# agent-charon/MinGraph-UNet

Hardware: AMD Instinct MI355X
Metric: segmented Mpix/sec, full MinGraph-UNet forward (U-Net + patch-graph GAT), 512x512 batch (higher is better)
Workload: dtype f32

## Files before the change

mingraph-unet_amd/csrc/convt_x3.hip:

```cpp
#include <hip/hip_runtime.h>
#include <stdint.h>

#include <algorithm>
#include <type_traits>

#include "common.h"
#include "pack_small.h"

namespace mgu {

typedef float f32x16 __attribute__((ext_vector_type(16)));
typedef float f32x4 __attribute__((ext_vector_type(4)));
typedef unsigned u32x4 __attribute__((ext_vector_type(4)));
typedef __bf16 bf16x8 __attribute__((ext_vector_type(8)));

namespace {

__device__ __forceinline__ void split3_pack(const float a, const float b, unsigned& p0, unsigned& p1, unsigned& p2) {
  const unsigned ua = __float_as_uint(a), ub = __float_as_uint(b);
  p0 = __builtin_amdgcn_perm(ub, ua, 0x07060302u);
  const float ra = a - __uint_as_float(ua & 0xffff0000u), rb = b - __uint_as_float(ub & 0xffff0000u);
  const unsigned va = __float_as_uint(ra), vb = __float_as_uint(rb);
  p1 = __builtin_amdgcn_perm(vb, va, 0x07060302u);
  const float sa = ra - __uint_as_float(va & 0xffff0000u), sb = rb - __uint_as_float(vb & 0xffff0000u);
  p2 = __builtin_amdgcn_perm(__float_as_uint(sb), __float_as_uint(sa), 0x07060302u);
}

__device__ __forceinline__ f32x16 mfma_bf16(const u32x4 a, const u32x4 b, const f32x16 c) {
  return __builtin_amdgcn_mfma_f32_32x32x16_bf16(__builtin_bit_cast(bf16x8, a), __builtin_bit_cast(bf16x8, b), c, 0, 0, 0);
}

__global__ void pack_convt_x3_kernel(const float* __restrict__ w, uint16_t* __restrict__ Wx, int Cin, int Cout) {
  pack_convt_x3_body(w, Wx, Cin, Cout, 0, blockIdx.x, gridDim.x);
}

__device__ __forceinline__ void lds_barrier() { asm volatile("s_waitcnt lgkmcnt(0)\n\ts_barrier" ::: "memory"); }

template <int MODE, int NI>
__global__ __launch_bounds__(256, 2) void convt2x2_x3_kernel(const float* __restrict__ in, const int ldin, const uint16_t* __restrict__ Wx,
                                                             const float* __restrict__ shift, float* __restrict__ out, const int M,
                                                             const int H, const int W, const int Cin, const int Cout, const int ldout,
                                                             const int coff, const int Hout, const int Wout, const int ntn,
                                                             const int nblocks) {
  constexpr int AP = 40, ABUF = 3 * 128 * AP;
  __shared__ __attribute__((aligned(16))) uint16_t As[2 * ABUF];
  __shared__ int rowoff[128];
  const int chunk = gridDim.x >> 3;
  const int lb = (blockIdx.x & 7) * chunk + (blockIdx.x >> 3);
  if (lb >= nblocks) return;
  const int nt = lb % ntn, mt = lb / ntn;
  const int tid = threadIdx.x, lane = tid & 63, wave = tid >> 6;
  const int wm = wave >> 1, wn = wave & 1, lr = lane & 31, lh = lane >> 5;
  const int bm0 = mt * 128;
  const int HW = H * W;
  long long pix0;
  {
    const int img = bm0 / HW, rem = bm0 - img * HW, y = rem / W;
    pix0 = ((long long)img * Hout + 2 * y) * Wout + 2 * (rem - y * W);
  }
  if (tid < 128) {
    const int m = bm0 + tid;
    int off = 0;
    if (m < M) {
      const int img = m / HW, rem = m - img * HW, y = rem / W, x = rem - y * W;
      off = (int)((((long long)img * Hout + 2 * y) * Wout + 2 * x - pix0) * ldout);
    }
    rowoff[tid] = off;
  }

  const int arow = tid >> 3, ach = (tid & 7) * 4;
  const float* aptr[4];
#pragma unroll
  for (int j = 0; j < 4; ++j) {
    const int m = min(bm0 + j * 32 + arow, M - 1);
    if (MODE == 0) {
      aptr[j] = in + (size_t)m * ldin + ach;
    } else {
      const int img = m / HW, rem = m - img * HW, y = rem / W, x = rem - y * W;
      aptr[j] = in + (((size_t)img * Hout + 2 * y) * Wout + 2 * x) * ldin + ach;
    }
  }
  const int nk = (MODE == 0 ? Cin : 4 * Cin) >> 5;
  const int spq = Cin >> 5;
  auto koff = [&](int s) -> int {
    if (MODE == 0) return s * 32;
    const int q = s / spq;
    return ((q >> 1) * Wout + (q & 1)) * ldin + (s - q * spq) * 32;
  };
  f32x4 areg[2][4];
  auto load_a = [&](int s, auto set_t) {
    constexpr int set = decltype(set_t)::value;
    const int ko = koff(s);
#pragma unroll
    for (int j = 0; j < 4; ++j) areg[set][j] = *reinterpret_cast<const f32x4*>(aptr[j] + ko);
  };
  auto store_a = [&](int buf, auto set_t) {
    constexpr int set = decltype(set_t)::value;
    uint16_t* const base = As + buf * ABUF + arow * AP + ach;
#pragma unroll
    for (int j = 0; j < 4; ++j) {
      unsigned p[3][2];
      split3_pack(areg[set][j][0], areg[set][j][1], p[0][0], p[1][0], p[2][0]);
      split3_pack(areg[set][j][2], areg[set][j][3], p[0][1], p[1][1], p[2][1]);
#pragma unroll
      for (int q = 0; q < 3; ++q) *reinterpret_cast<uint2*>(base + (q * 128 + j * 32) * AP) = uint2{p[q][0], p[q][1]};
    }
  };

  const int nt128 = NI == 2 ? nt : nt >> 1, sub0 = NI == 2 ? wn * 2 : (nt & 1) * 2 + wn;
  const u32x4* const bp = reinterpret_cast<const u32x4*>(Wx) + ((size_t)nt128 * (2 * nk) * 12 + sub0 * 3) * 64 + lane;
  u32x4 br[2][3 * NI];
  auto load_b = [&](int kk, auto buf_t) {
    constexpr int buf = decltype(buf_t)::value;
#pragma unroll
    for (int f = 0; f < 3 * NI; ++f) br[buf][f] = bp[((size_t)kk * 12 + f) * 64];
  };

  f32x16 acc[2][NI];
#pragma unroll
  for (int mi = 0; mi < 2; ++mi)
#pragma unroll
    for (int ni = 0; ni < NI; ++ni)
#pragma unroll
      for (int r = 0; r < 16; ++r) acc[mi][ni][r] = 0.f;

  const int aoff = (wm * 64 + lr) * AP + lh * 8;
  auto half_step = [&](int buf, int ss, auto bb_t) {
    constexpr int bb = decltype(bb_t)::value;
    u32x4 pa[2][3];
#pragma unroll
    for (int mi = 0; mi < 2; ++mi)
#pragma unroll
      for (int q = 0; q < 3; ++q)
        pa[mi][q] = *reinterpret_cast<const u32x4*>(As + buf * ABUF + (q * 128 + mi * 32) * AP + aoff + ss * 16);
#pragma unroll
    for (int mi = 0; mi < 2; ++mi)
#pragma unroll
      for (int ni = 0; ni < NI; ++ni) {
        f32x16 t = acc[mi][ni];
        t = mfma_bf16(pa[mi][2], br[bb][ni * 3 + 0], t);
        t = mfma_bf16(pa[mi][0], br[bb][ni * 3 + 2], t);
        t = mfma_bf16(pa[mi][1], br[bb][ni * 3 + 1], t);
        t = mfma_bf16(pa[mi][1], br[bb][ni * 3 + 0], t);
        t = mfma_bf16(pa[mi][0], br[bb][ni * 3 + 1], t);
        t = mfma_bf16(pa[mi][0], br[bb][ni * 3 + 0], t);
        acc[mi][ni] = t;
      }
  };
  using B0 = std::integral_constant<int, 0>;
  using B1 = std::integral_constant<int, 1>;
  const int nkk = 2 * nk;
  load_a(0, B0{});
  load_a(min(1, nk - 1), B1{});
  load_b(0, B0{});
  store_a(0, B0{});
  lds_barrier();
  auto second_half_and_stage = [&](int buf, auto bb_t, auto set_t) {
    half_step(buf, 1, bb_t);
    store_a(buf ^ 1, set_t);
#pragma unroll
    for (int k = 0; k < 12 * NI; ++k) {
      __builtin_amdgcn_sched_group_barrier(0x008, 1, 0);
      __builtin_amdgcn_sched_group_barrier(0x002, NI == 2 ? 4 : 8, 0);
    }
    __builtin_amdgcn_sched_group_barrier(0x200, 12, 0);
  };
  for (int s = 0; s < nk; s += 2) {
    load_a(min(s + 2, nk - 1), B0{});
    load_b(min(2 * s + 1, nkk - 1), B1{});
    __builtin_amdgcn_sched_barrier(0);
    half_step(0, 0, B0{});
    load_b(min(2 * s + 2, nkk - 1), B0{});
    __builtin_amdgcn_sched_barrier(0);
    second_half_and_stage(0, B1{}, B1{});
    __builtin_amdgcn_sched_barrier(0);
    lds_barrier();
    if (s + 1 >= nk) break;
    load_a(min(s + 3, nk - 1), B1{});
    load_b(min(2 * s + 3, nkk - 1), B1{});
    __builtin_amdgcn_sched_barrier(0);
    half_step(1, 0, B0{});
    load_b(min(2 * s + 4, nkk - 1), B0{});
    __builtin_amdgcn_sched_barrier(0);
    second_half_and_stage(1, B1{}, B0{});
    __builtin_amdgcn_sched_barrier(0);
    lds_barrier();
  }

  float* const tile_out = MODE == 0 ? out + (size_t)pix0 * ldout + coff : out + (size_t)bm0 * ldout + coff;
  const bool full_m = bm0 + 128 <= M;
  auto store_tile = [&](auto guarded_t) {
    constexpr bool GUARDED = decltype(guarded_t)::value;
#pragma unroll
    for (int ni = 0; ni < NI; ++ni) {
      const int n = nt * (64 * NI) + wn * (32 * NI) + ni * 32 + lr;
      int ncol = n;
      if (MODE == 0) {
        const int q = n / Cout;
        ncol = ((q >> 1) * Wout + (q & 1)) * ldout + (n - q * Cout);
      }
      const float sh = shift ? shift[n] : 0.f;
#pragma unroll
      for (int mi = 0; mi < 2; ++mi)
#pragma unroll
        for (int r = 0; r < 16; ++r) {
          const int rrow = wm * 64 + mi * 32 + (r & 3) + 8 * (r >> 2) + 4 * lh;
          const unsigned idx = (unsigned)((MODE == 0 ? rowoff[rrow] : rrow * ldout) + ncol);
          const float v = acc[mi][ni][r] + sh;
          if (!GUARDED) tile_out[idx] = v;
          else if (bm0 + rrow < M) tile_out[idx] = v;
        }
    }
  };
  if (full_m) store_tile(std::false_type{});
  else store_tile(std::true_type{});
}

}

size_t convt_x3_floats(int Cin, int Cout) { return (size_t)Cin * Cout * 6; }


namespace {

__global__ void pack_convt_x3_dgrad_kernel(const float* __restrict__ w, uint16_t* __restrict__ Wx, int Cin, int Cout) {
  pack_convt_x3_body(w, Wx, Cin, Cout, 1, blockIdx.x, gridDim.x);
}

}

size_t convt_x3_dgrad_floats(int Cin, int Cout) { return (size_t)((Cin + 127) / 128 * 128) * Cout * 6; }

hipError_t launch_pack_convt_x3_dgrad(const float* w, float* Wx, int Cin, int Cout, hipStream_t s) {
  if ((Cin & 63) || (Cout & 31)) return hipErrorInvalidValue;
  hipLaunchKernelGGL(pack_convt_x3_dgrad_kernel, dim3((unsigned)std::min<int64_t>(4096, ((int64_t)Cin * Cout * 4 + 255) / 256)), dim3(256), 0, s, w,
                     reinterpret_cast<uint16_t*>(Wx), Cin, Cout);
  return hipGetLastError();
}

hipError_t launch_convt_x3_dgrad(const IgemmDesc& d, hipStream_t s) {
  const bool wide = (d.N & 127) == 0;
  const int mtiles = (d.M + 127) / 128, ntn = d.N / (wide ? 128 : 64);
  const int nb = mtiles * ntn;
  const int chunk = (nb + 7) / 8;
  if (wide)
    hipLaunchKernelGGL((convt2x2_x3_kernel<1, 2>), dim3(chunk * 8), dim3(256), 0, s, d.in, d.ldin, reinterpret_cast<const uint16_t*>(d.wu),
                       (const float*)nullptr, d.out, d.M, d.H, d.W, d.Cp, d.N, d.ldout, d.coff, d.Hout, d.Wout, ntn, nb);
  else
    hipLaunchKernelGGL((convt2x2_x3_kernel<1, 1>), dim3(chunk * 8), dim3(256), 0, s, d.in, d.ldin, reinterpret_cast<const uint16_t*>(d.wu),
                       (const float*)nullptr, d.out, d.M, d.H, d.W, d.Cp, d.N, d.ldout, d.coff, d.Hout, d.Wout, ntn, nb);
  return hipGetLastError();
}

hipError_t launch_pack_convt_x3(const float* w, float* Wx, int Cin, int Cout, hipStream_t s) {
  if ((Cin & 15) || (Cout & 31)) return hipErrorInvalidValue;
  hipLaunchKernelGGL(pack_convt_x3_kernel, dim3((unsigned)std::min<int64_t>(4096, ((int64_t)Cin * Cout * 4 + 255) / 256)), dim3(256), 0, s, w, reinterpret_cast<uint16_t*>(Wx), Cin,
                     Cout);
  return hipGetLastError();
}

hipError_t launch_convt_x3(const IgemmDesc& d, hipStream_t s) {
  const int mtiles = (d.M + 127) / 128, ntn = d.N / 128;
  const int nb = mtiles * ntn;
  const int chunk = (nb + 7) / 8;
  hipLaunchKernelGGL((convt2x2_x3_kernel<0, 2>), dim3(chunk * 8), dim3(256), 0, s, d.in, d.ldin, reinterpret_cast<const uint16_t*>(d.wu), d.shift, d.out,
                     d.M, d.H, d.W, d.Cp, d.ct_cout, d.ldout, d.coff, d.Hout, d.Wout, ntn, nb);
  return hipGetLastError();
}

}
```

Baseline: 800.3.

## Make MODE-0 transposed-conv kernel persistent with prefetch of next tile during epilogue

The MODE-0 transposed-conv GEMM kernel becomes persistent. The grid is capped at about two workgroups per CU, and each workgroup walks tiles with a stride of gridDim. While the current tile's output is being stored, the next tile's A and B prologue loads and its A staging are issued. Row offsets are double-buffered in LDS, and B loads are shifted later within each step. The aim is to hide prologue latency and remove per-tile launch and tail overhead, at the cost of more register pressure and more complex control flow.

After: 801.4 (median of 6 runs). About the same (+0.1%).

```diff
diff --git a/mingraph-unet_amd/csrc/convt_x3.hip b/mingraph-unet_amd/csrc/convt_x3.hip
--- a/mingraph-unet_amd/csrc/convt_x3.hip
+++ b/mingraph-unet_amd/csrc/convt_x3.hip
@@ -2,6 +2,7 @@
 #include <stdint.h>
 
 #include <algorithm>
+#include <atomic>
 #include <type_traits>
 
 #include "common.h"
@@ -42,46 +43,54 @@
                                                              const int H, const int W, const int Cin, const int Cout, const int ldout,
                                                              const int coff, const int Hout, const int Wout, const int ntn,
                                                              const int nblocks) {
+  constexpr bool WALK = MODE == 0;
   constexpr int AP = 40, ABUF = 3 * 128 * AP;
   __shared__ __attribute__((aligned(16))) uint16_t As[2 * ABUF];
-  __shared__ int rowoff[128];
+  __shared__ int rowoff[WALK ? 2 : 1][128];
   const int chunk = gridDim.x >> 3;
-  const int lb = (blockIdx.x & 7) * chunk + (blockIdx.x >> 3);
+  int lb = (blockIdx.x & 7) * chunk + (blockIdx.x >> 3);
   if (lb >= nblocks) return;
-  const int nt = lb % ntn, mt = lb / ntn;
   const int tid = threadIdx.x, lane = tid & 63, wave = tid >> 6;
   const int wm = wave >> 1, wn = wave & 1, lr = lane & 31, lh = lane >> 5;
-  const int bm0 = mt * 128;
   const int HW = H * W;
-  long long pix0;
-  {
-    const int img = bm0 / HW, rem = bm0 - img * HW, y = rem / W;
-    pix0 = ((long long)img * Hout + 2 * y) * Wout + 2 * (rem - y * W);
-  }
-  if (tid < 128) {
-    const int m = bm0 + tid;
-    int off = 0;
-    if (m < M) {
-      const int img = m / HW, rem = m - img * HW, y = rem / W, x = rem - y * W;
-      off = (int)((((long long)img * Hout + 2 * y) * Wout + 2 * x - pix0) * ldout);
-    }
-    rowoff[tid] = off;
-  }
-
   const int arow = tid >> 3, ach = (tid & 7) * 4;
-  const float* aptr[4];
-#pragma unroll
-  for (int j = 0; j < 4; ++j) {
-    const int m = min(bm0 + j * 32 + arow, M - 1);
-    if (MODE == 0) {
-      aptr[j] = in + (size_t)m * ldin + ach;
-    } else {
-      const int img = m / HW, rem = m - img * HW, y = rem / W, x = rem - y * W;
-      aptr[j] = in + (((size_t)img * Hout + 2 * y) * Wout + 2 * x) * ldin + ach;
-    }
-  }
   const int nk = (MODE == 0 ? Cin : 4 * Cin) >> 5;
   const int spq = Cin >> 5;
+
+  int nt, bm0;
+  long long pix0;
+  const float* aptr[4];
+  const u32x4* bp;
+  auto start_tile = [&](const int t, const int rb) {
+    nt = __builtin_amdgcn_readfirstlane(t % ntn);
+    bm0 = __builtin_amdgcn_readfirstlane((t / ntn) * 128);
+    {
+      const int img = bm0 / HW, rem = bm0 - img * HW, y = rem / W;
+      pix0 = ((long long)img * Hout + 2 * y) * Wout + 2 * (rem - y * W);
+    }
+    if (tid < 128) {
+      const int m = bm0 + tid;
+      int off = 0;
+      if (m < M) {
+        const int img = m / HW, rem = m - img * HW, y = rem / W, x = rem - y * W;
+        off = (int)((((long long)img * Hout + 2 * y) * Wout + 2 * x - pix0) * ldout);
+      }
+      rowoff[rb][tid] = off;
+    }
+#pragma unroll
+    for (int j = 0; j < 4; ++j) {
+      const int m = min(bm0 + j * 32 + arow, M - 1);
+      if (MODE == 0) {
+        aptr[j] = in + (size_t)m * ldin + ach;
+      } else {
+        const int img = m / HW, rem = m - img * HW, y = rem / W, x = rem - y * W;
+        aptr[j] = in + (((size_t)img * Hout + 2 * y) * Wout + 2 * x) * ldin + ach;
+      }
+    }
+    const int nt128 = NI == 2 ? nt : nt >> 1, sub0 = NI == 2 ? wn * 2 : (nt & 1) * 2 + wn;
+    bp = reinterpret_cast<const u32x4*>(Wx) + ((size_t)nt128 * (2 * nk) * 12 + sub0 * 3) * 64 + lane;
+  };
+
   auto koff = [&](int s) -> int {
     if (MODE == 0) return s * 32;
     const int q = s / spq;
@@ -107,8 +116,6 @@
     }
   };
 
-  const int nt128 = NI == 2 ? nt : nt >> 1, sub0 = NI == 2 ? wn * 2 : (nt & 1) * 2 + wn;
-  const u32x4* const bp = reinterpret_cast<const u32x4*>(Wx) + ((size_t)nt128 * (2 * nk) * 12 + sub0 * 3) * 64 + lane;
   u32x4 br[2][3 * NI];
   auto load_b = [&](int kk, auto buf_t) {
     constexpr int buf = decltype(buf_t)::value;
@@ -117,13 +124,6 @@
   };
 
   f32x16 acc[2][NI];
-#pragma unroll
-  for (int mi = 0; mi < 2; ++mi)
-#pragma unroll
-    for (int ni = 0; ni < NI; ++ni)
-#pragma unroll
-      for (int r = 0; r < 16; ++r) acc[mi][ni][r] = 0.f;
-
   const int aoff = (wm * 64 + lr) * AP + lh * 8;
   auto half_step = [&](int buf, int ss, auto bb_t) {
     constexpr int bb = decltype(bb_t)::value;
@@ -150,11 +150,12 @@
   using B0 = std::integral_constant<int, 0>;
   using B1 = std::integral_constant<int, 1>;
   const int nkk = 2 * nk;
-  load_a(0, B0{});
-  load_a(min(1, nk - 1), B1{});
-  load_b(0, B0{});
-  store_a(0, B0{});
-  lds_barrier();
+  auto load_first = [&]() {
+    load_a(0, B0{});
+    load_a(min(1, nk - 1), B1{});
+    load_b(0, B0{});
+    if (WALK) load_b(1, B1{});
+  };
   auto second_half_and_stage = [&](int buf, auto bb_t, auto set_t) {
     half_step(buf, 1, bb_t);
     store_a(buf ^ 1, set_t);
@@ -165,55 +166,102 @@
     }
     __builtin_amdgcn_sched_group_barrier(0x200, 12, 0);
   };
-  for (int s = 0; s < nk; s += 2) {
-    load_a(min(s + 2, nk - 1), B0{});
-    load_b(min(2 * s + 1, nkk - 1), B1{});
+
+  auto step = [&](int s, auto buf_t) {
+    constexpr int buf = decltype(buf_t)::value;
+    load_a(min(s + 2, nk - 1), std::integral_constant<int, buf>{});
+    if (!WALK) load_b(min(2 * s + 1, nkk - 1), B1{});
     __builtin_amdgcn_sched_barrier(0);
-    half_step(0, 0, B0{});
+    half_step(buf, 0, B0{});
     load_b(min(2 * s + 2, nkk - 1), B0{});
     __builtin_amdgcn_sched_barrier(0);
-    second_half_and_stage(0, B1{}, B1{});
+    second_half_and_stage(buf, B1{}, std::integral_constant<int, buf ^ 1>{});
     __builtin_amdgcn_sched_barrier(0);
+    if (WALK) load_b(min(2 * s + 3, nkk - 1), B1{});
     lds_barrier();
-    if (s + 1 >= nk) break;
-    load_a(min(s + 3, nk - 1), B1{});
-    load_b(min(2 * s + 3, nkk - 1), B1{});
-    __builtin_amdgcn_sched_barrier(0);
-    half_step(1, 0, B0{});
-    load_b(min(2 * s + 4, nkk - 1), B0{});
-    __builtin_amdgcn_sched_barrier(0);
-    second_half_and_stage(1, B1{}, B0{});
-    __builtin_amdgcn_sched_barrier(0);
+  };
+
+  int rb = 0;
+  start_tile(lb, rb);
+  load_first();
+  store_a(0, B0{});
+  if (WALK) __builtin_amdgcn_s_waitcnt(0);
+  for (;;) {
+#pragma unroll
+    for (int mi = 0; mi < 2; ++mi)
+#pragma unroll
+      for (int ni = 0; ni < NI; ++ni)
+#pragma unroll
+        for (int r = 0; r < 16; ++r) acc[mi][ni][r] = 0.f;
     lds_barrier();
-  }
-
-  float* const tile_out = MODE == 0 ? out + (size_t)pix0 * ldout + coff : out + (size_t)bm0 * ldout + coff;
-  const bool full_m = bm0 + 128 <= M;
-  auto store_tile = [&](auto guarded_t) {
-    constexpr bool GUARDED = decltype(guarded_t)::value;
+    float sh[NI];
 #pragma unroll
     for (int ni = 0; ni < NI; ++ni) {
       const int n = nt * (64 * NI) + wn * (32 * NI) + ni * 32 + lr;
-      int ncol = n;
-      if (MODE == 0) {
-        const int q = n / Cout;
-        ncol = ((q >> 1) * Wout + (q & 1)) * ldout + (n - q * Cout);
-      }
-      const float sh = shift ? shift[n] : 0.f;
-#pragma unroll
-      for (int mi = 0; mi < 2; ++mi)
-#pragma unroll
-        for (int r = 0; r < 16; ++r) {
-          const int rrow = wm * 64 + mi * 32 + (r & 3) + 8 * (r >> 2) + 4 * lh;
-          const unsigned idx = (unsigned)((MODE == 0 ? rowoff[rrow] : rrow * ldout) + ncol);
-          const float v = acc[mi][ni][r] + sh;
-          if (!GUARDED) tile_out[idx] = v;
-          else if (bm0 + rrow < M) tile_out[idx] = v;
+      if (WALK) {
+        const float v = (shift ? shift : reinterpret_cast<const float*>(Wx))[n];
+        sh[ni] = shift ? v : 0.f;
+      } else {
+        sh[ni] = shift ? shift[n] : 0.f;
+      }
+    }
+    if (WALK) {
+      step(0, B0{});
+      for (int s = 1; s < nk; s += 2) {
+        step(s, B1{});
+        if (s + 1 >= nk) break;
+        step(s + 1, B0{});
+      }
+    } else {
+      for (int s = 0; s < nk; s += 2) {
+        step(s, B0{});
+        if (s + 1 >= nk) break;
+        step(s + 1, B1{});
+      }
+    }
+
+    const int cnt = nt, cbm0 = bm0;
+    float* const tile_out = MODE == 0 ? out + (size_t)pix0 * ldout + coff : out + (size_t)bm0 * ldout + coff;
+    const int* const crow = rowoff[rb];
+    auto store_tile = [&](auto guarded_t) {
+      constexpr bool GUARDED = decltype(guarded_t)::value;
+#pragma unroll
+      for (int ni = 0; ni < NI; ++ni) {
+        const int n = cnt * (64 * NI) + wn * (32 * NI) + ni * 32 + lr;
+        int ncol = n;
+        if (MODE == 0) {
+          const int q = n / Cout;
+          ncol = ((q >> 1) * Wout + (q & 1)) * ldout + (n - q * Cout);
         }
-    }
-  };
-  if (full_m) store_tile(std::false_type{});
-  else store_tile(std::true_type{});
+#pragma unroll
+        for (int mi = 0; mi < 2; ++mi)
+#pragma unroll
+          for (int r = 0; r < 16; ++r) {
+            const int rrow = wm * 64 + mi * 32 + (r & 3) + 8 * (r >> 2) + 4 * lh;
+            const unsigned idx = (unsigned)((MODE == 0 ? crow[rrow] : rrow * ldout) + ncol);
+            const float v = acc[mi][ni][r] + sh[ni];
+            if (!GUARDED) tile_out[idx] = v;
+            else if (cbm0 + rrow < M) tile_out[idx] = v;
+          }
+      }
+    };
+    if (cbm0 + 128 > M) {
+      store_tile(std::true_type{});
+      break;
+    }
+    int next = nblocks;
+    if (WALK) {
+      next = lb + (int)gridDim.x;
+      rb ^= 1;
+      start_tile(next < nblocks ? next : lb, rb);
+      load_first();
+      __builtin_amdgcn_sched_barrier(0);
+    }
+    store_tile(std::false_type{});
+    if (WALK) store_a(0, B0{});
+    if (next >= nblocks) break;
+    lb = next;
+  }
 }
 
 }
@@ -262,8 +310,19 @@
 hipError_t launch_convt_x3(const IgemmDesc& d, hipStream_t s) {
   const int mtiles = (d.M + 127) / 128, ntn = d.N / 128;
   const int nb = mtiles * ntn;
-  const int chunk = (nb + 7) / 8;
-  hipLaunchKernelGGL((convt2x2_x3_kernel<0, 2>), dim3(chunk * 8), dim3(256), 0, s, d.in, d.ldin, reinterpret_cast<const uint16_t*>(d.wu), d.shift, d.out,
+  static std::atomic<int> resident_of[64];
+  int dev = 0;
+  (void)hipGetDevice(&dev);
+  std::atomic<int>& slot = resident_of[dev >= 0 && dev < 64 ? dev : 0];
+  int resident = slot.load(std::memory_order_relaxed);
+  if (!resident) {
+    int cus = 256;
+    (void)hipDeviceGetAttribute(&cus, hipDeviceAttributeMultiprocessorCount, dev);
+    resident = std::max(8, cus * 2 / 8 * 8);
+    slot.store(resident, std::memory_order_relaxed);
+  }
+  const int nwg = std::min((nb + 7) / 8 * 8, std::max(resident, (ntn + 7) / 8 * 8));
+  hipLaunchKernelGGL((convt2x2_x3_kernel<0, 2>), dim3(nwg), dim3(256), 0, s, d.in, d.ldin, reinterpret_cast<const uint16_t*>(d.wu), d.shift, d.out,
                      d.M, d.H, d.W, d.Cp, d.ct_cout, d.ldout, d.coff, d.Hout, d.Wout, ntn, nb);
   return hipGetLastError();
 }
```
